# AIR-DISCOVER/Omni-PQ

Measured on AMD Instinct MI355X. Metric: scenes/sec fwd+bwd, 40k-pt ScanNet clouds, batch 8/GPU, higher is better.
Workload: dtype bf16; 1 GPU; BASELINE configs[1]: PQ_Transformer fwd+bwd, 40000-pt synthetic room scenes, batch 8/GPU, 3 input channels; global_batch=8, points=40000, parallelism=dp1, loss=sum of output means (SURVEY 8d)

## Files before the change

### include/omnipq_sa.h

```cpp
#ifndef OMNIPQ_SA_H
#define OMNIPQ_SA_H
#ifdef __cplusplus
extern "C" {

typedef struct omnipq_row_plan {
  const int *rows_dev;
  const void *row_w;
  const int *goff;
  long long rows;
  int gs;
  const float *pool_gamma;
} omnipq_row_plan;

#endif

int omnipq_sa_gather(int b, int n, int m, int s, int cin, int kpad, float inv_radius, const float *xyz,
                     const float *new_xyz, const int *idx, const void *feat_pm, void *X, const omnipq_row_plan *plan, void *stream);

int omnipq_sa_scatter(int b, int n, int m, int s, int cin, int kpad, float inv_radius, const int *idx,
                      const void *dX, float *dfeat_pm, float *dxyz, float *dnew_xyz, void *stream);

int omnipq_sa_build_csr(int b, int n, int m, int s, const int *idx, int *offsets, int *order, int *scratch,
                        const omnipq_row_plan *plan, void *stream);
int omnipq_sa_scatter_csr(int b, int n, int m, int s, int cin, int kpad, float inv_radius, const int *offsets,
// ... 59 lines not shown
                                      float *running_mean, float *running_var, const float *conv_bias, float *a_out,
                                      float *b_out, float *mean_out, float *invstd_out, const void *B, int ldb, void *C,
                                      int ldc, const float *bias, double *sums, float *workspace, int s, void *ymax,
                                      void *ymin, unsigned char *amax, unsigned char *amin, const omnipq_row_plan *plan, void *stream);
int omnipq_sa_pool_select(long long BM, int C, const void *ymax, const void *ymin, const unsigned char *amax,
                          const unsigned char *amin, const float *a, const float *bshift, float *out_f32, void *out_pm,
                          unsigned char *arg, void *ysel, void *stream);
int omnipq_sa_pool_select_finalize(long long BM, int C, const void *ymax, const void *ymin, const unsigned char *amax,
                                   const unsigned char *amin, const double *sums, double count, const float *gamma,
                                   const float *beta, float eps, float momentum, float *running_mean, float *running_var,
                                   float *a_out, float *b_out, float *mean_out, float *invstd_out, float *out_f32,
                                   void *out_pm, unsigned char *arg, void *ysel, const omnipq_row_plan *plan, void *stream);

int omnipq_sa_pool_bwd_stats_sel(long long BM, int C, const void *ysel, const float *mean, const float *invstd,
                                 const float *g_out, const void *out_pm, double *sums, int zeroed, void *stream);
int omnipq_sa_pool_bwd_stats_sel_hot(long long BM, int C, const void *ysel, const float *mean, const float *invstd,
                                     const float *g_out, const void *out_pm, double *sums, int zeroed, const float *a,
                                     const unsigned char *arg, unsigned *hot, void *stream);
int omnipq_gemm_tn_e16_affine(int M, int N, int P, const void *A, int lda, const void *B, int ldb, const float *ba,
                               const float *bb, float *C, float *workspace, float *colsum, const omnipq_row_plan *plan, void *stream);
int omnipq_gemm_tn_grouped(int nprob, const void *probs, float *workspace, void *stream);
int omnipq_gemm_nt_e16_f32(int M, int N, int K, const void *A, int lda, const void *B, int ldb, float *C, int ldc,
                            void *stream);
long long omnipq_sa_l1_rows_workspace_bytes(int b, int m, int s, int C);
int omnipq_sa_l1_rows(int b, int n, int m, int s, int C, float inv_radius, const float *xyz, const float *new_xyz,
                      const int *idx, const float *Z, const void *W1x, int ldw, const int *rows_dev, const int *unit_src,
                      const unsigned char *row_w, void *Y, void *Xrel, double *sums, void *workspace, void *tickets,
                      void *stream);
int omnipq_sa_scatter_rows_csr(int b, int n, int m, int s, int C, float inv_radius, const int *offsets, const int *order,
                               const void *dY, const void *dXr, const int *goff, int gs, float *dfeat32, void *dfeat16,
                               float *dxyz, float *dnew_xyz, void *stream);
void omnipq_tn_debug(int flags);
void omnipq_gemm_nt_small_tile_limit(int tiles);
int omnipq_tn_occupancy(int which);

int omnipq_sa_ball_plan(long long balls, int nsample, int gs, const int *idx, int *goff, int *rows_dev, void *row_w,
                        int *scratch, void *stream);
int omnipq_sa_ball_plan_src(long long balls, int nsample, int gs, const int *idx, int *goff, int *rows_dev, void *row_w,
                            int *unit_src, int *scratch, void *stream);

long long omnipq_gemm_nt_stats_workspace_floats(int M, int N);
int omnipq_gemm_nt_e16_stats(int M, int N, int K, const void *A, int lda, const void *B, int ldb, void *C,
                              int ldc, const float *bias, double *sums, float *workspace, const omnipq_row_plan *plan, void *stream);

int omnipq_gemm_nt_e16_bnbwd(int M, int N, int K, const void *A, int lda, const void *B, int ldb, void *C,
                              int ldc, const void *Y, const float *a, const float *b, const float *mean,
                              const float *invstd, double *sums, float *workspace, const omnipq_row_plan *plan, void *stream);

int omnipq_sa_xyz_moments(long long P, const void *X0, int ldx, double *mom, const omnipq_row_plan *plan, void *stream);
int omnipq_sa_xyz_stats(int C, const void *W0, int ldw0, const double *mom, double *sums, void *stream);
int omnipq_gemm_nt_e16_xyz_bnaffine(int M, int N, int K, const void *X0, int ldx, const void *W0, int ldw0,
                                     const double *fin_sums, double count, const float *gamma, const float *beta,
                                     float eps, float momentum, float *running_mean, float *running_var, float *a_out,
                                     float *b_out, float *mean_out, float *invstd_out, const void *B, int ldb, void *C,
                                     int ldc, double *sums, float *workspace, const omnipq_row_plan *plan, void *stream);
long long omnipq_gemm_nt_xyz_workspace_floats(int M, int N);
int omnipq_gemm_nt_e16_xyz_bnbwd(int M, int N, int K, const void *A, int lda, const void *B, int ldb, const void *X0,
                                  int ldx, const void *W0, int ldw0, const float *a, const float *b, const float *mean,
                                  const float *invstd, double *sums5, float *workspace, const omnipq_row_plan *plan, void *stream);
int omnipq_gemm_tn_e16_xyz_affine(int M, int N, int P, const void *A, int lda, const void *X0, int ldx, const void *W0,
                                   int ldw0, const float *ba, const float *bb, float *C, float *workspace, const omnipq_row_plan *plan, void *stream);
int omnipq_sa_xyz_bwd(int C, const void *W0, int ldw0, const double *mom, const double *sums5, const float *a,
                      const float *mean, const float *invstd, double inv_count, float *dW, void *stream);

int omnipq_colstats(long long P, int C, const void *Y, double *sums, void *stream);
int omnipq_colstats_z(long long P, int C, const void *Y, double *sums, void *stream);
// ... 105 lines not shown
```

### omni-pq_amd/csrc/gemm_bf16.hip

```cpp
#include <atomic>
#include <type_traits>

#include "common.h"

namespace omnipq {

typedef float f32x16 __attribute__((ext_vector_type(16)));
typedef float f32x4 __attribute__((ext_vector_type(4)));

constexpr int GBM = 128, GBN = 128, GBK = 32;
constexpr int GPITCH = 40;

struct GemmArgs {
  int M, N, K;
  int lda, ldb, ldc;
  int k_chunk;
  int m_tiles, n_tiles;
  int relu = 0;
  unsigned drop_thresh = 0, drop_salt = 0;
  float drop_keep_inv = 1.f;
  const unsigned long long *drop_seed = nullptr;
  const int *rows_dev = nullptr;
  const unsigned char *row_w = nullptr;
  int no_store = 0;
};
#ifndef OMNIPQ_DZ_WGS
#define OMNIPQ_DZ_WGS 3
#endif

__device__ __forceinline__ uint4 ldg16(const e16_t *p) { return *reinterpret_cast<const uint4 *>(p); }

#ifdef OMNIPQ_NT_TRACE
__device__ long long g_nt_trace[4096 * 8];
__device__ long long g_nt_real[4096 * 2];
__device__ __forceinline__ long long nt_now() {
  long long t;
  asm volatile("s_waitcnt vmcnt(0) lgkmcnt(0)\n\ts_memtime %0\n\ts_waitcnt lgkmcnt(0)" : "=s"(t) : : "memory");
  return t;
}
#define NT_STAMP(slot)                                                                    \
  {                                                                                       \
    const long long now_ = nt_now();                                                      \
    if (threadIdx.x == 0 && blockIdx.x < 4096) g_nt_trace[blockIdx.x * 8 + (slot)] = now_; \
    if ((slot) == 0 || (slot) == 7) {                                                     \
      const long long real_ = (long long)__builtin_amdgcn_s_memrealtime();                \
      if (threadIdx.x == 0 && blockIdx.x < 4096) g_nt_real[blockIdx.x * 2 + ((slot) == 7)] = real_; \
    }                                                                                     \
  }
#else
#define NT_STAMP(slot)
#endif

struct BnBwdEpilogue {
  const e16_t *Y;
  const float *a, *b, *mean, *invstd;
};

// ... 132 lines not shown
      dzw[i] = (float)g.row_w[ar];
      dzpf[i] = dz.unit_src[ar >> 3] * 8 + (ar & 7);
    }
  }

  f32x16 acc[NI][NI];
#pragma unroll
  for (int i = 0; i < NI; ++i)
#pragma unroll
    for (int j = 0; j < NI; ++j)
#pragma unroll
      for (int r = 0; r < 16; ++r) acc[i][j][r] = 0.f;

  float x0r[NI][3];
  if (XG == 2) {
    for (int c = tid; c < g.N; c += 256) {
      const uint2 w = *reinterpret_cast<const uint2 *>(xg.W0 + (size_t)c * xg.ldw);
      *w0_at(c) = f32x4{e16_lo(w.x), e16_hi(w.x),
                      e16_lo(w.y), 0.f};
    }
    __syncthreads();
  }
  if (XG == 1) {
#pragma unroll
    for (int i = 0; i < NI; ++i) {
      int ar = m0 + srow[i];
      ar = ar < Meff ? ar : Meff - 1;
      const uint2 v = *reinterpret_cast<const uint2 *>(xg.X0 + (size_t)ar * xg.ldx);
      x0r[i][0] = e16_lo(v.x);
      x0r[i][1] = e16_hi(v.x);
      x0r[i][2] = e16_lo(v.y);
    }
  }
  if (AFF) {
    const bool first = bid == 0 && blockIdx.z == 0;
    const int kaff = DZ ? g.K - GBK : g.K;
    for (int c = tid; c < kaff; c += 256) {
      float av, bv;
      if (aff.sums) {
        const double mu = aff.sums[c] / aff.count;
        double var = aff.sums[g.K + c] / aff.count - mu * mu;
        if (var < 0) var = 0;
        const float is = (float)(1.0 / sqrt(var + (double)aff.eps));
        av = aff.gamma[c] * is;
        bv = aff.beta[c] - (float)mu * av;
        if (first) {
          aff.a_out[c] = av;
          aff.b_out[c] = bv;
          aff.mean_out[c] = (float)mu;
          aff.invstd_out[c] = is;
          if (aff.running_mean) {
            const double unbiased = aff.count > 1 ? var * aff.count / (aff.count - 1) : var;
            const float shift = aff.conv_bias ? aff.conv_bias[c] : 0.f;
            aff.running_mean[c] = (1.f - aff.momentum) * aff.running_mean[c] + aff.momentum * ((float)mu + shift);
            aff.running_var[c] = (1.f - aff.momentum) * aff.running_var[c] + aff.momentum * (float)unbiased;
          }
        }
      } else {
        av = aff.a[c];
        bv = aff.b[c];
      }
      if (!PADW0) {
        *aff_at(0, c) = av;
        *aff_at(1, c) = bv;
      }
      if (XG == 1) {
        const uint2 w = *reinterpret_cast<const uint2 *>(xg.W0 + (size_t)c * xg.ldw);
// ... 66 lines not shown
        RA[i_].w = affine_relu_pair(RA[i_].w, fa4_[1][2], fb4_[1][2], fa4_[1][3], fb4_[1][3]);          \
      }                                                                                                 \
      }                                                                                                 \
    }                                                                                                   \
    _Pragma("unroll") for (int i_ = 0; i_ < NI; ++i_) {                                                 \
      *reinterpret_cast<uint4 *>(sa_ + srow[i_] * GPITCH + skc[i_] * 8) = RA[i_];                       \
      *reinterpret_cast<uint4 *>(sb_ + srow[i_] * GPITCH + skc[i_] * 8) = RB[i_];                       \
    }                                                                                                   \
  }

  const int frow = lane & 31, fk = (lane >> 5) * 8;
  auto mma_step = [&](int buf) {
    const e16_t *sa = stage + buf * (2 * T * GPITCH);
    const e16_t *sb = sa + T * GPITCH;
#pragma unroll
    for (int kk = 0; kk < 2; ++kk) {
      e16x8 fa[NI], fb[NI];
#pragma unroll
      for (int i = 0; i < NI; ++i) {
        fa[i] = *reinterpret_cast<const e16x8 *>(sa + (wm * (T / 2) + i * 32 + frow) * GPITCH + kk * 16 + fk);
        fb[i] = *reinterpret_cast<const e16x8 *>(sb + (wn * (T / 2) + i * 32 + frow) * GPITCH + kk * 16 + fk);
      }
#pragma unroll
      for (int i = 0; i < NI; ++i)
#pragma unroll
        for (int j = 0; j < NI; ++j)
          acc[i][j] = mfma_e16_32x32x16(fa[i], fb[j], acc[i][j]);
    }
  };

  if (KRES) {
    const int KP = nk * GBK + 8;
    e16_t *sa = stage, *sb = stage + T * KP;
    uint4 qa[kResMaxSteps], qb[kResMaxSteps];
#pragma unroll
    for (int kt = 0; kt < kResMaxSteps; ++kt)
      if (kt < nk) {
        qa[kt] = ldg16(ga[0] + kt * GBK);
        qb[kt] = ldg16(gb[0] + kt * GBK);
      }
#pragma unroll
    for (int kt = 0; kt < kResMaxSteps; ++kt)
      if (kt < nk) {
        if (AFF) {
          const int k0 = kbeg + kt * GBK + skc[0] * 8;
          const f32x4 fa0 = *reinterpret_cast<const f32x4 *>(aff_at(0, k0)), fa1 = *reinterpret_cast<const f32x4 *>(aff_at(0, k0 + 4));
          const f32x4 fb0 = *reinterpret_cast<const f32x4 *>(aff_at(1, k0));
          const f32x4 fb1 = *reinterpret_cast<const f32x4 *>(aff_at(1, k0 + 4));
          qa[kt].x = affine_relu_pair(qa[kt].x, fa0[0], fb0[0], fa0[1], fb0[1]);
          qa[kt].y = affine_relu_pair(qa[kt].y, fa0[2], fb0[2], fa0[3], fb0[3]);
          qa[kt].z = affine_relu_pair(qa[kt].z, fa1[0], fb1[0], fa1[1], fb1[1]);
          qa[kt].w = affine_relu_pair(qa[kt].w, fa1[2], fb1[2], fa1[3], fb1[3]);
        }
        *reinterpret_cast<uint4 *>(sa + srow[0] * KP + kt * GBK + skc[0] * 8) = qa[kt];
        *reinterpret_cast<uint4 *>(sb + srow[0] * KP + kt * GBK + skc[0] * 8) = qb[kt];
      }
    __syncthreads();
    const e16_t *pa = sa + (wm * (T / 2) + frow) * KP + fk;
    const e16_t *pb = sb + (wn * (T / 2) + frow) * KP + fk;
    for (int kt = 0; kt < nk; ++kt) {
#pragma unroll
      for (int kk = 0; kk < 2; ++kk) {
        const e16x8 fa = *reinterpret_cast<const e16x8 *>(pa + kt * GBK + kk * 16);
        const e16x8 fb = *reinterpret_cast<const e16x8 *>(pb + kt * GBK + kk * 16);
        acc[0][0] = mfma_e16_32x32x16(fa, fb, acc[0][0]);
      }
    }
    __syncthreads();
  } else {
  if (nk > 0) {
    OMNIPQ_LOAD_TILES(ra, rb, 0)
    OMNIPQ_STORE_TILES(ra, rb, 0, 0)
  }
  __syncthreads();
  NT_STAMP(2);

  for (int kt = 0; kt < nk; ++kt) {
    const int buf = kt & 1;
    if (kt + 1 < nk) OMNIPQ_LOAD_TILES(ra, rb, kt + 1)
    mma_step(buf);
    if (kt + 1 < nk) OMNIPQ_STORE_TILES(ra, rb, buf ^ 1, kt + 1)
    __syncthreads();
  }
  if (DZ) {
    const int nk2 = dz.C3 / GBK;
    unsigned dzt[NI];
    const unsigned *dzh[NI];
    const e16_t *gb2[NI];
#pragma unroll
// ... 91 lines not shown
#pragma unroll
          for (int r = 0; r < 16; r += 2) {
            float mine0 = HAS_BIAS ? acc[i][j][r] + bcol[j] : acc[i][j][r];
            float mine1 = HAS_BIAS ? acc[i][j][r + 1] + bcol[j] : acc[i][j][r + 1];
            if (STATS == 0 && g.relu) {
              mine0 = __builtin_fmaxf(mine0, 0.f);
              mine1 = __builtin_fmaxf(mine1, 0.f);
              if (g.drop_thresh) {
                const unsigned e0 = (unsigned)(m0 + wm * (T / 2) + i * 32 + (r & 3) + 8 * (r >> 2) + crow0) * (unsigned)g.ldc +
                                    (unsigned)(n0 + wn * (T / 2) + j * 32 + ccol);
                mine0 = dec_hash(e0, rd_seed) >= g.drop_thresh ? mine0 * g.drop_keep_inv : 0.f;
                mine1 = dec_hash(e0 + (unsigned)g.ldc, rd_seed) >= g.drop_thresh ? mine1 * g.drop_keep_inv : 0.f;
              }
            }
            const unsigned mine = pack_e16x2(mine0, mine1);
            const unsigned other = (unsigned)__builtin_amdgcn_mov_dpp((int)mine, 0xB1, 0xF, 0xF, true);
            cbase[(i * 32 + (r & 3) + 8 * (r >> 2)) * (CP / 2) + j * 16] = __builtin_amdgcn_perm(other, mine, pair_sel);
          }
    };
    if (bias)
      pack_tile(std::true_type{});
    else
      pack_tile(std::false_type{});
    const e16_t *ct = reinterpret_cast<const e16_t *>(smem);
    __syncthreads();
    NT_STAMP(4);
    e16_t *C = reinterpret_cast<e16_t *>(Cout);
    float cs[8], cs2[8];
#pragma unroll
    for (int e = 0; e < 8; ++e) cs[e] = cs2[e] = 0.f;
    float av[8], bv[8], mu[8], is[8];
    float cx[XG == 2 ? 3 : 1][8];
    f32x4 wcol[XG == 2 ? 8 : 1];
    if (STATS == 3 || STATS == 4) {
      int c0 = n0 + (tid % PIECES) * 8;
      c0 = c0 < g.N ? c0 : 0;
#pragma unroll
      for (int e = 0; e < 8; ++e) {
        av[e] = bn.a[c0 + e];
        bv[e] = bn.b[c0 + e];
        mu[e] = bn.mean[c0 + e];
        is[e] = bn.invstd[c0 + e];
        if (XG == 2) {
          wcol[e] = *w0_at(c0 + e);
          cx[0][e] = cx[1][e] = cx[2][e] = 0.f;
        }
      }
    }
    constexpr int ITERS = T * PIECES / 256;
    uint4 ypre[(STATS >= 3 && XG != 2) ? ITERS : 1];
    if (STATS >= 3 && XG != 2) {
#pragma unroll
      for (int it = 0; it < ITERS; ++it) {
        const int q = tid + it * 256;
        const int row = q / PIECES, piece = q % PIECES;
        int gr = m0 + row, gc = n0 + piece * 8;
        gr = gr < Meff ? gr : Meff - 1;
        gc = gc < g.N ? gc : 0;
        ypre[it] = *reinterpret_cast<const uint4 *>(bn.Y + (size_t)gr * g.ldc + gc);
      }
    }
#pragma unroll
    for (int it = 0; it < ITERS; ++it) {
      const int q = tid + it * 256;
      const int row = q / PIECES, piece = q % PIECES;
      const int gr = m0 + row, gc = n0 + piece * 8;
      if (gr < Meff && gc < g.N) {
        const uint4 v = *reinterpret_cast<const uint4 *>(ct + row * CP + piece * 8);
        if (STATS == 5) {
          const uint4 hv = ypre[it];
          const unsigned w[4] = {v.x, v.y, v.z, v.w}, hw[4] = {hv.x, hv.y, hv.z, hv.w};
          unsigned o[4];
#pragma unroll
          for (int e = 0; e < 4; ++e) {
            const float d0 = e16_lo(w[e]), d1 = e16_hi(w[e]);
            const float h0 = e16_lo(hw[e]), h1 = e16_hi(hw[e]);
            o[e] = pack_e16x2(h0 > 0.f ? d0 * g.drop_keep_inv : 0.f, h1 > 0.f ? d1 * g.drop_keep_inv : 0.f);
          }
          *reinterpret_cast<uint4 *>(C + (size_t)gr * g.ldc + gc) = make_uint4(o[0], o[1], o[2], o[3]);
          continue;
        }
        if (XG != 2 && !((STATS == 1 || STATS == 2) && g.no_store))
          *reinterpret_cast<uint4 *>(C + (size_t)gr * g.ldc + gc) = v;
        if (XG == 2) {
// ... 423 lines not shown
  OMNIPQ_LAUNCH_CHECK();
  const long long n4 = (long long)M * N / 4;
  splitk_reduce_bf16_kernel<<<(unsigned)((n4 + 255) / 256), 256, 0, (hipStream_t)stream>>>(
      n4, N, used, reinterpret_cast<const f32x4 *>(workspace), bias, (e16_t *)C);
  OMNIPQ_LAUNCH_CHECK();
  return OMNIPQ_OK;
}

static int g_small_tile_limit = 256;
extern "C" void omnipq_gemm_nt_small_tile_limit(int tiles) { g_small_tile_limit = tiles; }
static bool gemm_nt_small_tiles(int M, int N) {
  return (long long)((M + 127) / 128) * ((N + 127) / 128) <= g_small_tile_limit;
}

static void plan_rows(omnipq::GemmArgs &g) {
  const omnipq::RowPlan &rp = omnipq::row_plan();
  if (rp.rows_dev && rp.rows == g.M && g.m_tiles > kStatsDirectTiles) {
    g.rows_dev = rp.rows_dev;
    g.row_w = rp.row_w;
  }
}

static int stats_reduce(const omnipq::GemmArgs &g, int ns, float *workspace, double *sums, void *stream) {
  int slabs = g.m_tiles / 64;
  if (slabs > 128) slabs = 128;
  if (slabs < 1) slabs = 1;
  omnipq::partial_reduce_kernel<<<dim3((ns * g.N + 255) / 256, slabs), 256, 0, (hipStream_t)stream>>>(
      g.m_tiles, ns * g.N, workspace, sums, g.rows_dev);
  OMNIPQ_LAUNCH_CHECK();
  return OMNIPQ_OK;
}

static bool gemm_nt_kres(int K) { return K <= omnipq::kResMaxSteps * omnipq::GBK; }

static thread_local omnipq::HeldLaunch t_held;
static std::atomic<long long> t_pairs_launched{0};
namespace omnipq {
HeldLaunch &held_launch() { return t_held; }
void count_pair_launch() { ++t_pairs_launched; }
}
struct HeldSmallBlob {
  omnipq::SmallProblem p;
  int lds;
};

static void flush_held() {
  if (t_held.held) omnipq::release_held(t_held);
}

template <int STATS, bool AFF>
static void launch_small_single(const omnipq::SmallProblem &p, int lds, hipStream_t stream) {
  using namespace omnipq;
  auto kern = gemm_nt_kernel<false, STATS, AFF, 64, 0, true>;
  static const hipError_t prepared = hipFuncSetAttribute(reinterpret_cast<const void *>(kern),
                                                         hipFuncAttributeMaxDynamicSharedMemorySize, 96 * 1024);
  (void)prepared;
  kern<<<gemm_nt_grid(p.g), 256, lds, stream>>>(p.g, p.A, p.B, p.C, p.bias, p.stats, p.bn, p.aff, PoolOut(), XyzGen(), DzGen());
}

template <int STATS, bool AFF>
static void held_single(const void *blob, hipStream_t stream) {
  HeldSmallBlob q;
  __builtin_memcpy(&q, blob, sizeof(q));
  launch_small_single<STATS, AFF>(q.p, q.lds, stream);
}

// ... 2 lines not shown
  using namespace omnipq;
  if (n == 2) {
    auto kern = gemm_nt_pair_kernel<STATS, AFF>;
    static const hipError_t prepared = hipFuncSetAttribute(reinterpret_cast<const void *>(kern),
                                                           hipFuncAttributeMaxDynamicSharedMemorySize, 96 * 1024);
    (void)prepared;
    const int n0 = (int)gemm_nt_grid(q[0].p.g).x, n1 = (int)gemm_nt_grid(q[1].p.g).x;
    kern<<<dim3(n0 + n1), 256, q[0].lds > q[1].lds ? q[0].lds : q[1].lds, stream>>>(q[0].p, q[1].p, n0);
    return 1;
  }
  if constexpr (!AFF && (STATS == 0 || STATS == 3)) {
    auto kern = gemm_nt_group_kernel<STATS, AFF>;
    static const hipError_t prepared = hipFuncSetAttribute(reinterpret_cast<const void *>(kern),
                                                           hipFuncAttributeMaxDynamicSharedMemorySize, 96 * 1024);
    (void)prepared;
    NtGroupArgs a;
    a.n = n;
    int wgs = 0, lds = 0;
    for (int i = 0; i < n; ++i) {
      const SmallProblem &p = q[i].p;
      a.item[i] = NtGroupItem{p.g, p.A, p.B, p.C, p.bias, p.stats, p.bn, wgs};
      wgs += (int)gemm_nt_grid(p.g).x;
      lds = q[i].lds > lds ? q[i].lds : lds;
    }
    kern<<<dim3(wgs), 256, lds, stream>>>(a);
    return 1;
  } else {
    for (int i = 0; i < n; ++i) launch_small_single<STATS, AFF>(q[i].p, q[i].lds, stream);
    return 0;
  }
}

template <int STATS, bool AFF>
static void launch_small(const omnipq::GemmArgs &g, const void *A, const void *B, void *C, const float *bias, void *stats,
                         const omnipq::BnBwdEpilogue &bn, const omnipq::AffineIn &aff, void *stream) {
  using namespace omnipq;
  if (gemm_nt_kres(g.K)) {
    int lds = 2 * 64 * (g.K + 8) * 2;
    if (lds < 20480) lds = 20480;
    const HeldSmallBlob q{SmallProblem{g, (const e16_t *)A, (const e16_t *)B, C, bias, stats, bn, aff}, lds};
    const bool consumed = hold_or_pair(
        q, STATS * 2 + (AFF ? 1 : 0), (hipStream_t)stream, &held_single<STATS, AFF>,
        [&](const HeldSmallBlob *recs, int n) { return launch_small_group<STATS, AFF>(recs, n, (hipStream_t)stream); });
    if (!consumed) launch_small_single<STATS, AFF>(q.p, lds, (hipStream_t)stream);
  } else {
    flush_held();
    gemm_nt_kernel<false, STATS, AFF, 64><<<gemm_nt_grid(g), 256, 0, (hipStream_t)stream>>>(
        g, (const e16_t *)A, (const e16_t *)B, C, bias, stats, bn, aff, PoolOut(), XyzGen());
  }
}

extern "C" void omnipq_pair_hold(void) {
  if (!t_held.held || t_held.group) t_held.armed = true;
}

extern "C" int omnipq_pair_group(int n) {
  flush_held();
  t_held.armed = false;
  t_held.group = 0;
  if (n < 1 || n > omnipq::kHeldMax) return OMNIPQ_EINVAL;
  t_held.group = n;
  return OMNIPQ_OK;
}

extern "C" int omnipq_pair_held(void) { return t_held.held; }

extern "C" long long omnipq_pair_flush(void) {
  flush_held();
  t_held.armed = false;
  t_held.group = 0;
// ... 399 lines not shown
```

### omni-pq_amd/pointnet2/rows_mlp.py

```python
import collections
import ctypes
import functools
import os
import typing

import torch

import dropout_state
import sa_fused
from sa_fused import E16, _call, _gemm_nt_bnbwd, _gemm_nt_stats, _gemm_tn, _lib, _p, _round_up, _world, prep_weight, unprep_wgrad, zeros_f32

_FUSE_ACT = True


class Layer:

    def __init__(self, weight, bias=None, bn=None, relu_dropout=None):
        self.weight, self.bias, self.bn, self.relu_dropout = weight, bias, bn, relu_dropout


def enabled():
    return os.environ.get("OMNIPQ_ROWS", "rows") != "torch"


# ... 67 lines not shown
def stack_route(training, N, cin, layers, no_grad=False):
    if no_grad and not training and EVAL_CHAIN and len(layers) >= 2 and \
            all(cout % 32 == 0 for cout, kind in layers if kind == "bn") and \
            eval_chain_ok(cin, tuple(_round_up(cout, 32) for cout, _ in layers)):
        return StackRoute(False, tuple(LayerRoute(kind, "lds" if l else "input", "chain", "folded" if kind == "bn" else "",
                                                  "epilogue" if kind == "act" else "", "", "", "")
                                       for l, (_, kind) in enumerate(layers)))
    L, K, out = len(layers), _round_up(cin, 32), []
    for l, (cout, kind) in enumerate(layers):
        Cp = _round_up(cout, 32)
        feed = "input" if l == 0 else "yab" if out[-1].finalize == "consumer" else "stored"
        if kind == "bn" and training:
            gemm = "stats"
        elif kind == "act" and feed != "yab" and _FUSE_ACT and K < 1024 and N * Cp < (1 << 32):
            gemm = "relu_dropout"
        else:
            gemm = "plain"
        finalize = ""
        if kind == "bn":
            finalize = "running" if not training else \
                "consumer" if (l < L - 1 and sa_fused.affine_pays(N, layers[l + 1][0])) else "launch"
        below = layers[l - 1][1] if l else None
        dgrad = "input" if l == 0 else "bnbwd" if below == "bn" else \
            "mask" if (below == "act" and _FUSE_ACT and Cp < 1024) else "plain"
        out.append(LayerRoute(kind, feed, gemm, finalize, "" if kind != "act" else "epilogue" if gemm == "relu_dropout" else "pass",
                              dgrad, "" if kind != "bn" else "above" if l < L - 1 else "own", ""))
        K = Cp
    for l, r in enumerate(out):
        if r.kind == "act":
            out[l] = r._replace(bwd_act="above" if (l < L - 1 and out[l + 1].dgrad == "mask") else "pass")
    return StackRoute(bool(training), tuple(out))


class _L:
    __slots__ = ("act", "K", "C", "Cp", "Wp", "Wt", "wk", "a", "b", "mean", "invstd", "Y", "X", "has_bias", "fin")


def _hold(lead):
    if lead:
        _lib.omnipq_pair_hold()


def _drain(gen):
    assert not _lib.omnipq_pair_held(), "rows_mlp: a held pair launch leaked into a lone stack"
    try:
        while True:
            next(gen)
    except StopIteration as done:
        return done.value


def _lockstep(*gens):
    n = len(gens)
    out = [None] * n
    alive = [True] * n
    assert not _lib.omnipq_pair_held(), "rows_mlp: a pair launch was still held when a lockstep run started"
    outer, sa_fused.PairStats.active = sa_fused.PairStats.active, sa_fused.PairStats() if n == 2 else None
    try:
        while any(alive):
            if n > 2:
                _lib.omnipq_pair_group(sum(alive))
            for i in range(n):
                if not alive[i]:
                    continue
                held = _lib.omnipq_pair_held()
                try:
                    next(gens[i])
                except StopIteration as done:
                    out[i], alive[i] = done.value, False
                if i < n - 1 and _lib.omnipq_pair_held() != held + 1:
                    _lib.omnipq_pair_flush()
            _lib.omnipq_pair_flush()
    finally:
        sa_fused.PairStats.active = outer
        _lib.omnipq_pair_flush()
    assert not _lib.omnipq_pair_held()
    return out


class _Ctx:
    __slots__ = ("route", "layers", "X0", "geom", "wshapes", "nbias", "targets", "in_dtype", "padded")



def _input_rows(x, N, cin, K):
    cached = getattr(x, "omnipq_rows_in", None)
    if cached is not None and cached[0] == x._version and cached[1].shape == (N, K):
        return cached[1]
    if K == cin:
        X = x.detach().to(E16.dtype).contiguous()
    elif x.dtype in (torch.float32, E16.dtype) and x.stride(1) == 1:
        X = torch.empty((N, K), device=x.device, dtype=E16.dtype)
        _call(_lib.omnipq_pad_rows_e16, x, N, cin, K, x.stride(0), _p(x), int(x.dtype == torch.float32), _p(X))
    else:
        X = torch.nn.functional.pad(x.detach().to(E16.dtype), (0, K - cin))
    if X.data_ptr() != x.data_ptr() and not x.requires_grad:
        try:
            x.omnipq_rows_in = (x._version, X)
        except Exception:
            pass
    return X


def _new_layer(W, bias, K, act, training):
    lay = _L()
    W2 = W.detach().reshape(W.shape[0], -1)
    lay.C, lay.wk = W2.shape
    lay.K, lay.Cp = K, _round_up(lay.C, 32)
    lay.has_bias, lay.act, lay.fin = bias is not None, act, None
    lay.Wp, lay.Wt = prep_weight(W2, lay.Cp, K, transpose=training, persistent=sa_fused.is_persistent(W))
    return lay


def _padded_bias(bias, Cp):
# ... 68 lines not shown
    world = _world() if (training and spec.sync) else 1
    route = stack_route(training, N, cin, tuple((params[4 * l].shape[0], _kind(spec.layers[l])) for l in range(L)))
    X0 = X = _input_rows(x, N, cin, _round_up(cin, 32))
    K = X.shape[1]
    layers = []
    for l, r in enumerate(route.layers):
        W, bias, gamma, beta = params[4 * l:4 * l + 4]
        lay = _new_layer(W, bias, K, spec.layers[l] if r.kind == "act" else None, training)
        if r.kind == "bn" and lay.Cp != lay.C:
            raise RuntimeError("RowsMLP: BatchNorm widths must be multiples of 32")
        sums, slot = sa_fused.pair_sums(lead, 2, lay.C, dev, world) if r.gemm == "stats" else (None, None)
        bp = _padded_bias(bias, lay.Cp) if (lay.has_bias and r.kind != "bn") else None
        _hold(lead)
        lay.Y = _GEMM[r.gemm](lay, X, layers[-1] if r.feed == "yab" else None, N, bp, sums)
        yield
        if r.kind == "bn":
            if training:
                sa_fused.pair_allreduce(sums, slot, lead, world)
            X = _FINALIZE[r.finalize](lay, N, float(N) * world, sums, spec.layers[l], bias, gamma, beta)
            if training:
                sa_fused.bump(spec.layers[l].num_batches_tracked)
        else:
            if r.act == "pass":
                _call(_lib.omnipq_relu_dropout, lay.Y, N * lay.Cp, _p(lay.Y), lay.act.p, _p(lay.act.seed), lay.act.salt)
            X = lay.X = lay.Y
        K = lay.Cp
        layers.append(lay)
    ctx.route, ctx.layers, ctx.X0, ctx.geom = route, layers, X0, (N, cin, world)
    ctx.wshapes = [tuple(params[4 * l].shape) for l in range(L)]
    ctx.nbias = [0 if params[4 * l + 1] is None else params[4 * l + 1].shape[0] for l in range(L)]
    ctx.targets = [(sa_fused.grad_target(params[4 * l]),
                    None if params[4 * l + 1] is None else sa_fused.grad_target(params[4 * l + 1]))
                   for l in range(L)] if training else None
    ctx.in_dtype, ctx.padded = x.dtype, spec.padded
    last = layers[-1]
    return X if (spec.padded or last.Cp == last.C) else X[:, :last.C]



def _layer_kind(lay):
    return "bn" if lay.bn is not None else "act" if lay.relu_dropout is not None else "plain"


def _chain_route(x, layers, training):
    if training or torch.is_grad_enabled() or x.dim() != 2:
        return None
    route = stack_route(False, x.shape[0], x.shape[1], tuple((lay.weight.shape[0], _layer_kind(lay)) for lay in layers), no_grad=True)
    return route if route.layers[0].gemm == "chain" else None


def _infer(x, layers, route, padded):
    global eval_chain_uses
    N, cin = x.shape
    x = x.detach()
    if x.dtype not in (torch.float32, E16.dtype) or x.stride(1) != 1:
        x = x.to(E16.dtype).contiguous()
    L = len(layers)
    recs = (_InferLayer * L)()
    keep = []
    K = _round_up(cin, 32)
    for lay, r, rec in zip(layers, route.layers, recs):
        nl = _new_layer(lay.weight, lay.bias, K, None, False)
        if r.kind == "bn":
            bn = lay.bn
            vecs = [v.detach().float().contiguous() for v in (bn.weight, bn.bias, bn.running_mean, bn.running_var)]
            rec.gamma, rec.beta, rec.running_mean, rec.running_var = (v.data_ptr() for v in vecs)
# ... 40 lines not shown
    wt, bt = ctx.targets[l] if (dfr is not None and ctx.targets is not None) else (None, None)
    if wt is not None and needs_input_grad[3 + 4 * l] and (
            not want_bias or (sa_fused.bias_target_ok(bt, lay.C, lay.Cp) and needs_input_grad[4 + 4 * l])):
        dfr.add(dcur, Xin, lay.Cp, lay.K, N, wt, sa_fused.Crop(lay.C, lay.wk), bt if want_bias else None, below)
        return
    bsum = None
    if want_bias:
        bsum = zeros_f32(lay.Cp, dcur.device)
        grads[4 * l + 1] = bsum[:ctx.nbias[l]]
    dWp = _gemm_tn(dcur, Xin, lay.Cp, lay.K, N, colsum=bsum, below=below)
    grads[4 * l] = unprep_wgrad(dWp, lay.C, lay.wk, 0, ctx.wshapes[l])


def _dgrad_bnbwd(lay, under, dcur, N, sums):
    return _gemm_nt_bnbwd(dcur, lay.Wt, N, lay.K, lay.Cp, under, sums)


def _dgrad_mask(lay, under, dcur, N, sums):
    dprev = torch.empty((N, lay.K), device=dcur.device, dtype=E16.dtype)
    _call(_lib.omnipq_gemm_nt_e16_mask, dcur, N, lay.K, lay.Cp, _p(dcur), lay.Cp, _p(lay.Wt), lay.Cp, _p(dprev), lay.K,
          _p(under.Y), under.act.p)
    return dprev


def _dgrad_plain(lay, under, dcur, N, sums):
    dprev = torch.empty((N, lay.K), device=dcur.device, dtype=E16.dtype)
    sa_fused.gemm_nt_into(dcur, lay.Wt, dprev, N, lay.K, lay.Cp)
    return dprev


_DGRAD = {"bnbwd": _dgrad_bnbwd, "mask": _dgrad_mask, "plain": _dgrad_plain, "input": _dgrad_plain}


def _backward_program(ctx, lead, g, needs_input_grad):
    route, layers = ctx.route, ctx.layers
    if not route.training and any(r.kind == "bn" for r in route.layers):
        raise RuntimeError("RowsMLP: backward through eval-mode BatchNorm is not supported")
    N, cin, world = ctx.geom
    L = len(layers)
    dev = g.device
    grads = [None] * (4 * L)
    dcur, owned = _output_grad(g, layers[-1], N, ctx.padded)
    dx = None
    sums = slot = None
    dfr = sa_fused.deferred_wgrads.active
    for l in range(L - 1, -1, -1):
        lay, r = layers[l], route.layers[l]
        below = layers[l - 1] if r.feed == "yab" else None
        Xin = ctx.X0 if r.feed == "input" else layers[l - 1].Y if r.feed == "yab" else layers[l - 1].X
        if r.kind == "bn":
            if r.bwd_stats == "own":
                sums, slot = sa_fused.pair_sums(lead, 3, lay.C, dev, world)
                _bn_bwd_stats(lay, dcur, N, sums)
                if sa_fused.PairStats.active is not None and (world > 1 or sa_fused._FORCE_COLLECTIVES):
                    yield
            assert sums is not None
            dst = dcur if owned else torch.empty_like(dcur)
            _hold(lead)
            grads[4 * l + 2], grads[4 * l + 3] = sa_fused.bn_backward_apply(dcur, lay, N, lay.C, float(N) * world, sums, world,
                                                                            out=dst, pair=(slot, lead))
            yield
            dcur, owned = dst, True
            if lay.has_bias:
                grads[4 * l + 1] = zeros_f32(lay.C, dev)
        elif r.bwd_act == "pass":
            dst = dcur if owned else torch.empty_like(dcur)
            _act_bwd(lay, dcur, dst, N)
            dcur, owned = dst, True
        _weight_grad(ctx, l, dcur, Xin, below, dfr, needs_input_grad, grads)
        sums = slot = None
        if r.dgrad == "input" and not needs_input_grad[0]:
            break
        if r.dgrad == "bnbwd":
            sums, slot = sa_fused.pair_sums(lead, 3, lay.K, dev, world)
        _hold(lead)
        dprev = _DGRAD[r.dgrad](lay, layers[l - 1] if l else None, dcur, N, sums)
        yield
        if l > 0:
            dcur, owned = dprev, True
        else:
            dx = dprev[:, :cin].to(ctx.in_dtype)
    ctx.layers = None
    return (dx, None, None, *grads)


class RowsMLP(torch.autograd.Function):
    @staticmethod
    def forward(ctx, x, spec, training, *params):
        ctx.e16 = E16.dtype
        return _drain(_forward_program(ctx, False, x, spec, training, params))

    @staticmethod
    def backward(ctx, g):
        E16.select(ctx.e16)
        return _drain(_backward_program(ctx, False, g, ctx.needs_input_grad))


class RowsMLPPair(torch.autograd.Function):

    @staticmethod
    def forward(ctx, xa, spec_a, xb, spec_b, training, n_a, *params):
        ctx.e16 = E16.dtype
        ctx.a, ctx.b, ctx.n_a = _Ctx(), _Ctx(), n_a
        ctx.set_materialize_grads(False)
        ya, yb = _lockstep(_forward_program(ctx.a, True, xa, spec_a, training, params[:n_a]),
                           _forward_program(ctx.b, False, xb, spec_b, training, params[n_a:]))
        return ya, yb

    @staticmethod
    def backward(ctx, ga, gb):
        E16.select(ctx.e16)
        nig, n_a = ctx.needs_input_grad, ctx.n_a
        nig_a = (nig[0], False, False) + tuple(nig[6:6 + n_a])
        nig_b = (nig[2], False, False) + tuple(nig[6 + n_a:])
        if ga is None and gb is None:
            return (None,) * len(nig)
        if ga is None or gb is None:
            outs = []
            for c, g, n in ((ctx.a, ga, nig_a), (ctx.b, gb, nig_b)):
                outs.append(_drain(_backward_program(c, False, g, n)) if g is not None else (None,) * len(n))
            oa, ob = outs
        else:
            oa, ob = _lockstep(*tape_programs(ctx, ga, gb, nig_a, nig_b))
        return (oa[0], None, ob[0], None, None, None) + tuple(oa[3:]) + tuple(ob[3:])


def _spec_of(x_rows, layers, training, padded):
    spec, params = [], []
    for lay in layers:
        bn = lay.bn
        if bn is None and lay.relu_dropout is not None:
            p = float(lay.relu_dropout) if training else 0.0
            spec.append(ActSpec(p, dropout_state.seed(x_rows.device) if p > 0 else None, dropout_state.next_salt() if p > 0 else 0))
        else:
            spec.append(None if bn is None else
                        BnSpec(bn.running_mean, bn.running_var, bn.num_batches_tracked, float(bn.momentum), float(bn.eps)))
        params += [lay.weight, lay.bias, None if bn is None else bn.weight, None if bn is None else bn.bias]
    bns = [lay.bn for lay in layers if lay.bn is not None]
    sync = bool(bns) and all(bool(sa_fused.bn_syncs(bn)) for bn in bns)
    return StackSpec(tuple(spec), bool(padded), sync), params


def run_pair(xa, layers_a, xb, layers_b, training, padded=False, eval_chain=False):
    if eval_chain:
        ra, rb = _chain_route(xa, layers_a, training), _chain_route(xb, layers_b, training)
        if ra is not None and rb is not None:
            return _infer(xa, layers_a, ra, padded), _infer(xb, layers_b, rb, padded)
    spec_a, params_a = _spec_of(xa, layers_a, training, padded)
    spec_b, params_b = _spec_of(xb, layers_b, training, padded)
    return RowsMLPPair.apply(xa, spec_a, xb, spec_b, bool(training), len(params_a), *params_a, *params_b)


class _Taped:
    saved_tensors = ()

# ... 23 lines not shown
```

### omni-pq_amd/pointnet2/sa_fused.py

```python
import collections
import ctypes
import functools
import os
import threading
import typing
import weakref

import torch
import torch.distributed as dist

import pointnet2_utils
import wgrads
from wgrads import Crop, bias_target_ok, cat_params, grad_target, joint_params

_ext = pointnet2_utils._load_ext()
_lib = _ext._lib
E16 = _ext.E16
if os.environ.get("OMNIPQ_TN_DEBUG"):
    _lib.omnipq_tn_debug(int(os.environ["OMNIPQ_TN_DEBUG"]))


def _p(t):
    return ctypes.c_void_p(t.data_ptr() if t is not None else 0)

# ... 422 lines not shown
        _call(_lib.omnipq_gemm_tn_e16_colsum, A, M, N, P, _p(A), M, _p(B), N, _p(C), _p(ws), _p(colsum))
    return C


_TnProblem = _ext.struct("omnipq_tn_problem")


def empty_f32(shape, device):
    return torch.empty(shape, device=device, dtype=torch.float32)


def _plan_buffer(b, dev):
    shape, device = ((b.numel,), dev) if b.param is None else (b.param.shape, b.param.device)
    if b.kind == "empty":
        return empty_f32(shape, device)
    if b.kind == "pooled":
        return zeros_f32(b.numel, device).view(shape)
    return torch.zeros(shape, device=device, dtype=torch.float32)


class deferred_wgrads:
    active = None

    def __init__(self, on_early_flush=None):
        self.on_early_flush = on_early_flush

    def __enter__(self):
        if deferred_wgrads.active is not None:
            raise RuntimeError("deferred_wgrads blocks do not nest")
        self.items = []
        self.sa_items = []
        self.ln_items = []
        self.dz_items = []
        self.producers = set()
        self._inflight = []
        self._assign = []
        self._side_streams = []
        deferred_wgrads.active = self
        return self

    def _note_producer(self, t):
        if t.is_cuda:
            self.producers.add(torch.cuda.current_stream(t.device))

    def add_layernorm(self, part, blocks, C, gamma, beta):
        self._note_producer(part)
        self.ln_items.append((part, blocks, C, gamma, beta))

    def add(self, dY, X, M, N, P, wt, crop, bt, below=None):
        wgrads._refuse_ddp(wt)
        self._note_producer(dY)
        self.items.append(wgrads.Item(dY, X, M, N, P, wt, crop, bt, None if below is None else (below.a, below.b)))

    def add_sa(self, dY, X, M, N, P, wt, crop, below=None, blk=None):
        wgrads._refuse_ddp(wt)
        self._note_producer(dY)
        self.sa_items.append(wgrads.Item(dY, X, M, N, P, wt, crop, None, None if below is None else (below.a, below.b), blk))

    def add_dz(self, args, wt, stage):
        wgrads._refuse_ddp(wt)
        self._note_producer(args[0])
        self.dz_items.append((args, wt, stage))

    def __exit__(self, et, ev, tb):
        deferred_wgrads.active = None
        global COLLECTIVES_LAST_STEP, _COLLECTIVES_MARK
        COLLECTIVES_LAST_STEP, _COLLECTIVES_MARK = COLLECTIVES - _COLLECTIVES_MARK, COLLECTIVES
        if et is None:
            self._wait_producers(None)
            self.flush()
        for st in self._side_streams:
            torch.cuda.current_stream(st.device).wait_stream(st)
        if et is None:
            for param, g in self._assign:
                self._accumulate(param, g)
        self.items = None
        self.sa_items = None
        self.dz_items = None
        self.ln_items = None
        self._inflight = None
        self._assign = None
        self._side_streams = None
        return False

    def _wait_producers(self, stream):
        for ps in self.producers:
            st = stream if stream is not None else torch.cuda.current_stream(ps.device)
            if ps != st:
                st.wait_stream(ps)

    def flush_on(self, stream):
        if not self.items and not self.ln_items:
            return
        cur = torch.cuda.current_stream(stream.device)
        stream.wait_stream(cur)
        self._wait_producers(stream)
        self._inflight.extend(self.items)
        self._inflight.extend(self.ln_items)
        if stream not in self._side_streams:
            self._side_streams.append(stream)
        with torch.cuda.stream(stream):
            self.flush()
            self.items = []
            self.ln_items = []
            if self.on_early_flush is not None:
                self.on_early_flush(self)

    def _flush_layernorms(self):
        todo, self.ln_items = self.ln_items, []
        for i0 in range(0, len(todo), 32):
            chunk = todo[i0:i0 + 32]
            n = len(chunk)
            dev = chunk[0][0].device
            flat = zeros_f32(sum(2 * it[2] for it in chunk), dev)
            parts = (ctypes.c_void_p * n)(*[it[0].data_ptr() for it in chunk])
            blocks = (ctypes.c_int * n)(*[it[1] for it in chunk])
            chans = (ctypes.c_int * n)(*[it[2] for it in chunk])
            outs, off = (ctypes.c_void_p * n)(), 0
            for i, (_, _, C, gamma, beta) in enumerate(chunk):
                outs[i] = flat.data_ptr() + 4 * off
                self._assign.append((gamma, flat[off:off + C].view(gamma.shape)))
                self._assign.append((beta, flat[off + C:off + 2 * C].view(beta.shape)))
                off += 2 * C
            _call(_lib.omnipq_layernorm_param_reduce, flat, n, parts, blocks, chans, outs)
            self._inflight.extend(chunk)

    def flush(self):
        if self.ln_items:
            self._flush_layernorms()
        if self.items:
            self._flush_items(self.items)
        if deferred_wgrads.active is None:
            self._flush_sa()

    def _flush_sa(self):
        if self.sa_items:
            items, self.sa_items = self.sa_items, []
            with _tagged("@sa"):
                self._flush_items(items)
            self._inflight.extend(items)
        if self.dz_items:
            todo, self.dz_items = self.dz_items, []
            for args, wt, stage in todo:
                Y2, below, hot, plan, S, C3, C2, P, alpha, beta, Wp = args
                with _tagged("@sa", stage), _row_plan(plan, P):
                    buf = last_wgrad_dz(Y2, below, hot, plan, S, C3, C2, P, alpha, beta, Wp)
                self._assign.append((wt.param, buf.view(wt.param.shape)))
            self._inflight.extend(todo)

    def _flush_items(self, items):
        dev = items[0].dY.device
        plan = wgrads.place(items)
        bufs = [_plan_buffer(b, dev) for b in plan.buffers]

        def span(s):
            return bufs[s.buf].view(-1)[s.off:s.off + s.n]

        probs = (_TnProblem * len(items))()
        for q, it, pr in zip(probs, items, plan.problems):
            q.rows_dev = 0 if it.blk is None else it.blk.rows_dev.data_ptr()
# ... 868 lines not shown
```

Measured before the change: 1080 scenes/s.

## Defer leaf RowsMLP backwards to end of backward and prefetch K-resident GEMM operands

Two independent changes. In the K-resident small GEMM, operand tiles, BN-affine statistics and epilogue Y/scale values are now loaded into registers before the affine-parameter computation and its barrier, so global-load latency overlaps that setup. In Python, the backward of leaf RowsMLP stacks (no input gradient, single device) is deferred to an autograd end-of-backward callback, and several stacks are run together in lockstep groups so their small launches can be paired. The deferral adds bookkeeping for parameter-gradient assignment and stream producers, and the register prefetch raises register pressure, which may reduce occupancy.

```diff
diff --git a/include/omnipq_sa.h b/include/omnipq_sa.h
--- a/include/omnipq_sa.h
+++ b/include/omnipq_sa.h
@@ -115,6 +115,7 @@
                                float *dxyz, float *dnew_xyz, void *stream);
 void omnipq_tn_debug(int flags);
 void omnipq_gemm_nt_small_tile_limit(int tiles);
+void omnipq_gemm_nt_kres_overlap(int on);
 int omnipq_tn_occupancy(int which);
 
 int omnipq_sa_ball_plan(long long balls, int nsample, int gs, const int *idx, int *goff, int *rows_dev, void *row_w,
diff --git a/omni-pq_amd/csrc/gemm_bf16.hip b/omni-pq_amd/csrc/gemm_bf16.hip
--- a/omni-pq_amd/csrc/gemm_bf16.hip
+++ b/omni-pq_amd/csrc/gemm_bf16.hip
@@ -23,6 +23,7 @@
   const int *rows_dev = nullptr;
   const unsigned char *row_w = nullptr;
   int no_store = 0;
+  int kres_overlap = 0;
 };
 #ifndef OMNIPQ_DZ_WGS
 #define OMNIPQ_DZ_WGS 3
@@ -221,7 +222,102 @@
       x0r[i][2] = e16_lo(v.y);
     }
   }
-  if (AFF) {
+  constexpr int KQ = kResMaxSteps;
+  constexpr bool KEPI = KRES && STATS == 3;
+  const bool kres_early = KRES && g.kres_overlap;
+  uint4 qa[KQ], qb[KQ];
+  float eav[KEPI ? 8 : 1], ebv[KEPI ? 8 : 1], emu[KEPI ? 8 : 1], eis[KEPI ? 8 : 1];
+  uint4 eypre[KEPI ? T * (T / 8) / 256 : 1];
+  constexpr int NC = AFF ? (kResMaxSteps * GBK + 255) / 256 : 1;
+  double ts0[NC], ts1[NC];
+  float tg[NC], tb[NC], trm[NC], trv[NC], tcb[NC];
+  if (AFF && KRES && kres_early) {
+    const bool first = bid == 0 && blockIdx.z == 0;
+#pragma unroll
+    for (int i = 0; i < NC; ++i) {
+      const int c = tid + i * 256;
+      tcb[i] = 0.f;
+      if (c < g.K) {
+        if (aff.sums) {
+          ts0[i] = aff.sums[c];
+          ts1[i] = aff.sums[g.K + c];
+          tg[i] = aff.gamma[c];
+          tb[i] = aff.beta[c];
+          if (first && aff.running_mean) {
+            trm[i] = aff.running_mean[c];
+            trv[i] = aff.running_var[c];
+            if (aff.conv_bias) tcb[i] = aff.conv_bias[c];
+          }
+        } else {
+          tg[i] = aff.a[c];
+          tb[i] = aff.b[c];
+        }
+      }
+    }
+  }
+  if (KRES && kres_early) {
+#pragma unroll
+    for (int kt = 0; kt < KQ; ++kt)
+      if (kt < nk) {
+        qa[kt] = ldg16(ga[0] + kt * GBK);
+        qb[kt] = ldg16(gb[0] + kt * GBK);
+      }
+    if (KEPI) {
+      int c0 = n0 + (tid % PIECES) * 8;
+      c0 = c0 < g.N ? c0 : 0;
+#pragma unroll
+      for (int it = 0; it < T * PIECES / 256; ++it) {
+        const int q = tid + it * 256;
+        int gr = m0 + q / PIECES, gc = n0 + (q % PIECES) * 8;
+        gr = gr < Meff ? gr : Meff - 1;
+        gc = gc < g.N ? gc : 0;
+        eypre[it] = *reinterpret_cast<const uint4 *>(bn.Y + (size_t)gr * g.ldc + gc);
+      }
+#pragma unroll
+      for (int e = 0; e < 8; ++e) {
+        eav[e] = bn.a[c0 + e];
+        ebv[e] = bn.b[c0 + e];
+        emu[e] = bn.mean[c0 + e];
+        eis[e] = bn.invstd[c0 + e];
+      }
+    }
+  }
+  if (AFF && KRES && kres_early) {
+    const bool first = bid == 0 && blockIdx.z == 0;
+#pragma unroll
+    for (int i = 0; i < NC; ++i) {
+      const int c = tid + i * 256;
+      if (c < g.K) {
+        float av, bv;
+        if (aff.sums) {
+          const double mu = ts0[i] / aff.count;
+          double var = ts1[i] / aff.count - mu * mu;
+          if (var < 0) var = 0;
+          const float is = (float)(1.0 / sqrt(var + (double)aff.eps));
+          av = tg[i] * is;
+          bv = tb[i] - (float)mu * av;
+          if (first) {
+            aff.a_out[c] = av;
+            aff.b_out[c] = bv;
+            aff.mean_out[c] = (float)mu;
+            aff.invstd_out[c] = is;
+            if (aff.running_mean) {
+              const double unbiased = aff.count > 1 ? var * aff.count / (aff.count - 1) : var;
+              const float shift = tcb[i];
+              aff.running_mean[c] = (1.f - aff.momentum) * trm[i] + aff.momentum * ((float)mu + shift);
+              aff.running_var[c] = (1.f - aff.momentum) * trv[i] + aff.momentum * (float)unbiased;
+            }
+          }
+        } else {
+          av = tg[i];
+          bv = tb[i];
+        }
+        *aff_at(0, c) = av;
+        *aff_at(1, c) = bv;
+      }
+    }
+    __syncthreads();
+  } else if (AFF) {
     const bool first = bid == 0 && blockIdx.z == 0;
     const int kaff = DZ ? g.K - GBK : g.K;
     for (int c = tid; c < kaff; c += 256) {
@@ -354,29 +450,35 @@
   if (KRES) {
     const int KP = nk * GBK + 8;
     e16_t *sa = stage, *sb = stage + T * KP;
-    uint4 qa[kResMaxSteps], qb[kResMaxSteps];
-#pragma unroll
-    for (int kt = 0; kt < kResMaxSteps; ++kt)
-      if (kt < nk) {
-        qa[kt] = ldg16(ga[0] + kt * GBK);
-        qb[kt] = ldg16(gb[0] + kt * GBK);
-      }
-#pragma unroll
-    for (int kt = 0; kt < kResMaxSteps; ++kt)
-      if (kt < nk) {
-        if (AFF) {
-          const int k0 = kbeg + kt * GBK + skc[0] * 8;
-          const f32x4 fa0 = *reinterpret_cast<const f32x4 *>(aff_at(0, k0)), fa1 = *reinterpret_cast<const f32x4 *>(aff_at(0, k0 + 4));
-          const f32x4 fb0 = *reinterpret_cast<const f32x4 *>(aff_at(1, k0));
-          const f32x4 fb1 = *reinterpret_cast<const f32x4 *>(aff_at(1, k0 + 4));
-          qa[kt].x = affine_relu_pair(qa[kt].x, fa0[0], fb0[0], fa0[1], fb0[1]);
-          qa[kt].y = affine_relu_pair(qa[kt].y, fa0[2], fb0[2], fa0[3], fb0[3]);
-          qa[kt].z = affine_relu_pair(qa[kt].z, fa1[0], fb1[0], fa1[1], fb1[1]);
-          qa[kt].w = affine_relu_pair(qa[kt].w, fa1[2], fb1[2], fa1[3], fb1[3]);
+    auto store_all = [&]() {
+#pragma unroll
+      for (int kt = 0; kt < kResMaxSteps; ++kt)
+        if (kt < nk) {
+          if (AFF) {
+            const int k0 = kbeg + kt * GBK + skc[0] * 8;
+            const f32x4 fa0 = *reinterpret_cast<const f32x4 *>(aff_at(0, k0)), fa1 = *reinterpret_cast<const f32x4 *>(aff_at(0, k0 + 4));
+            const f32x4 fb0 = *reinterpret_cast<const f32x4 *>(aff_at(1, k0));
+            const f32x4 fb1 = *reinterpret_cast<const f32x4 *>(aff_at(1, k0 + 4));
+            qa[kt].x = affine_relu_pair(qa[kt].x, fa0[0], fb0[0], fa0[1], fb0[1]);
+            qa[kt].y = affine_relu_pair(qa[kt].y, fa0[2], fb0[2], fa0[3], fb0[3]);
+            qa[kt].z = affine_relu_pair(qa[kt].z, fa1[0], fb1[0], fa1[1], fb1[1]);
+            qa[kt].w = affine_relu_pair(qa[kt].w, fa1[2], fb1[2], fa1[3], fb1[3]);
+          }
+          *reinterpret_cast<uint4 *>(sa + srow[0] * KP + kt * GBK + skc[0] * 8) = qa[kt];
+          *reinterpret_cast<uint4 *>(sb + srow[0] * KP + kt * GBK + skc[0] * 8) = qb[kt];
         }
-        *reinterpret_cast<uint4 *>(sa + srow[0] * KP + kt * GBK + skc[0] * 8) = qa[kt];
-        *reinterpret_cast<uint4 *>(sb + srow[0] * KP + kt * GBK + skc[0] * 8) = qb[kt];
-      }
+    };
+    if (kres_early) {
+      store_all();
+    } else {
+#pragma unroll
+      for (int kt = 0; kt < kResMaxSteps; ++kt)
+        if (kt < nk) {
+          qa[kt] = ldg16(ga[0] + kt * GBK);
+          qb[kt] = ldg16(gb[0] + kt * GBK);
+        }
+      store_all();
+    }
     __syncthreads();
     const e16_t *pa = sa + (wm * (T / 2) + frow) * KP + fk;
     const e16_t *pb = sb + (wn * (T / 2) + frow) * KP + fk;
@@ -534,7 +636,13 @@
     float av[8], bv[8], mu[8], is[8];
     float cx[XG == 2 ? 3 : 1][8];
     f32x4 wcol[XG == 2 ? 8 : 1];
-    if (STATS == 3 || STATS == 4) {
+    if (KEPI && kres_early) {
+#pragma unroll
+      for (int e = 0; e < 8; ++e) {
+        const int s = KEPI ? e : 0;
+        av[e] = eav[s], bv[e] = ebv[s], mu[e] = emu[s], is[e] = eis[s];
+      }
+    } else if (STATS == 3 || STATS == 4) {
       int c0 = n0 + (tid % PIECES) * 8;
       c0 = c0 < g.N ? c0 : 0;
 #pragma unroll
@@ -551,7 +659,10 @@
     }
     constexpr int ITERS = T * PIECES / 256;
     uint4 ypre[(STATS >= 3 && XG != 2) ? ITERS : 1];
-    if (STATS >= 3 && XG != 2) {
+    if (KEPI && kres_early) {
+#pragma unroll
+      for (int it = 0; it < ITERS; ++it) ypre[KEPI ? it : 0] = eypre[KEPI ? it : 0];
+    } else if (STATS >= 3 && XG != 2) {
 #pragma unroll
       for (int it = 0; it < ITERS; ++it) {
         const int q = tid + it * 256;
@@ -1041,6 +1152,8 @@
 }
 
 static bool gemm_nt_kres(int K) { return K <= omnipq::kResMaxSteps * omnipq::GBK; }
+static int g_kres_overlap = 1;
+extern "C" void omnipq_gemm_nt_kres_overlap(int on) { g_kres_overlap = on != 0; }
 
 static thread_local omnipq::HeldLaunch t_held;
 static std::atomic<long long> t_pairs_launched{0};
@@ -1109,10 +1222,12 @@
 }
 
 template <int STATS, bool AFF>
-static void launch_small(const omnipq::GemmArgs &g, const void *A, const void *B, void *C, const float *bias, void *stats,
+static void launch_small(const omnipq::GemmArgs &g_in, const void *A, const void *B, void *C, const float *bias, void *stats,
                          const omnipq::BnBwdEpilogue &bn, const omnipq::AffineIn &aff, void *stream) {
   using namespace omnipq;
+  GemmArgs g = g_in;
   if (gemm_nt_kres(g.K)) {
+    g.kres_overlap = g_kres_overlap;
     int lds = 2 * 64 * (g.K + 8) * 2;
     if (lds < 20480) lds = 20480;
     const HeldSmallBlob q{SmallProblem{g, (const e16_t *)A, (const e16_t *)B, C, bias, stats, bn, aff}, lds};
diff --git a/omni-pq_amd/pointnet2/rows_mlp.py b/omni-pq_amd/pointnet2/rows_mlp.py
--- a/omni-pq_amd/pointnet2/rows_mlp.py
+++ b/omni-pq_amd/pointnet2/rows_mlp.py
@@ -123,6 +123,18 @@
     return StackRoute(bool(training), tuple(out))
 
 
+DEFER_LEAF_BACKWARD = True
+_LEAF_GROUP_MAX = 14
+
+
+def leaf_backward_route(defer, block, input_grad, targets_ok, ddp_refused, world, force_collectives):
+    if not (defer and block) or input_grad or not targets_ok or ddp_refused:
+        return "now"
+    if world != 1 or force_collectives:
+        return "now"
+    return "deferred"
+
+
 class _L:
     __slots__ = ("act", "K", "C", "Cp", "Wp", "Wt", "wk", "a", "b", "mean", "invstd", "Y", "X", "has_bias", "fin")
 
@@ -170,7 +182,7 @@
 
 
 class _Ctx:
-    __slots__ = ("route", "layers", "X0", "geom", "wshapes", "nbias", "targets", "in_dtype", "padded")
+    __slots__ = ("route", "layers", "X0", "geom", "wshapes", "nbias", "targets", "in_dtype", "padded", "leaf")
 
 
 
@@ -305,6 +317,8 @@
     ctx.targets = [(sa_fused.grad_target(params[4 * l]),
                     None if params[4 * l + 1] is None else sa_fused.grad_target(params[4 * l + 1]))
                    for l in range(L)] if training else None
+    ctx.leaf = [tuple(params[4 * l + 1:4 * l + 4]) if r.kind == "bn" else None for l, r in enumerate(route.layers)] \
+        if training else None
     ctx.in_dtype, ctx.padded = x.dtype, spec.padded
     last = layers[-1]
     return X if (spec.padded or last.Cp == last.C) else X[:, :last.C]
@@ -411,7 +425,7 @@
 _DGRAD = {"bnbwd": _dgrad_bnbwd, "mask": _dgrad_mask, "plain": _dgrad_plain, "input": _dgrad_plain}
 
 
-def _backward_program(ctx, lead, g, needs_input_grad):
+def _backward_program(ctx, lead, g, needs_input_grad, dfr=None):
     route, layers = ctx.route, ctx.layers
     if not route.training and any(r.kind == "bn" for r in route.layers):
         raise RuntimeError("RowsMLP: backward through eval-mode BatchNorm is not supported")
@@ -422,7 +436,7 @@
     dcur, owned = _output_grad(g, layers[-1], N, ctx.padded)
     dx = None
     sums = slot = None
-    dfr = sa_fused.deferred_wgrads.active
+    dfr = dfr if dfr is not None else sa_fused.deferred_wgrads.active
     for l in range(L - 1, -1, -1):
         lay, r = layers[l], route.layers[l]
         below = layers[l - 1] if r.feed == "yab" else None
@@ -463,6 +477,66 @@
     return (dx, None, None, *grads)
 
 
+
+def _leaf_targets_ok(ctx, nig):
+    if ctx.targets is None or ctx.leaf is None:
+        return False
+    for l, (lay, r) in enumerate(zip(ctx.layers, ctx.route.layers)):
+        wt, bt = ctx.targets[l]
+        if wt is None or not nig[3 + 4 * l]:
+            return False
+        if r.kind == "bn":
+            for j, p in enumerate(ctx.leaf[l]):
+                if p is not None and not (isinstance(p, torch.nn.Parameter) and p.requires_grad and nig[4 + 4 * l + j]):
+                    return False
+        elif lay.has_bias and not (sa_fused.bias_target_ok(bt, lay.C, lay.Cp) and nig[4 + 4 * l]):
+            return False
+    return True
+
+
+def _leaf_ddp_refused(ctx):
+    ids = sa_fused.wgrads._DDP_PARAM_IDS
+    if not ids:
+        return False
+    params = [p for wt, bt in ctx.targets for t in (wt, bt) if t is not None for p in t.params]
+    params += [p for leaf in ctx.leaf if leaf is not None for p in leaf if p is not None]
+    return any(id(p) in ids for p in params)
+
+
+def _leaf_deferred(ctxs, nigs):
+    dfr = sa_fused.deferred_wgrads.active
+    for c, nig in zip(ctxs, nigs):
+        block = dfr is not None and c.targets is not None
+        if leaf_backward_route(DEFER_LEAF_BACKWARD, block, nig[0], block and _leaf_targets_ok(c, nig),
+                               block and _leaf_ddp_refused(c), max(c.geom[2], _world()),
+                               sa_fused._FORCE_COLLECTIVES) != "deferred":
+            return None
+    return dfr
+
+
+class LeafBackward(typing.NamedTuple):
+    ctx: object
+    g: torch.Tensor
+    nig: tuple
+    e16: object
+
+
+def run_leaf_backwards(dfr, leaves):
+    before = int(_lib.omnipq_pair_flush())
+    for i0 in range(0, len(leaves), _LEAF_GROUP_MAX):
+        chunk = leaves[i0:i0 + _LEAF_GROUP_MAX]
+        E16.select(chunk[0].e16)
+        progs = [_backward_program(lf.ctx, i + 1 < len(chunk), lf.g, lf.nig, dfr) for i, lf in enumerate(chunk)]
+        outs = _lockstep(*progs) if len(progs) > 1 else [_drain(progs[0])]
+        for lf, out in zip(chunk, outs):
+            for l, leaf in enumerate(lf.ctx.leaf):
+                for j, p in enumerate(leaf or ()):
+                    gp = out[3 + 4 * l + 1 + j]
+                    if p is not None and gp is not None:
+                        dfr.assign(p, gp.view(p.shape))
+    return int(_lib.omnipq_pair_flush()) - before
+
+
 class RowsMLP(torch.autograd.Function):
     @staticmethod
     def forward(ctx, x, spec, training, *params):
@@ -472,7 +546,12 @@
     @staticmethod
     def backward(ctx, g):
         E16.select(ctx.e16)
-        return _drain(_backward_program(ctx, False, g, ctx.needs_input_grad))
+        nig = ctx.needs_input_grad
+        dfr = _leaf_deferred((ctx,), (nig,))
+        if dfr is not None:
+            dfr.add_leaves([LeafBackward(ctx, g, tuple(nig), ctx.e16)])
+            return (None,) * len(nig)
+        return _drain(_backward_program(ctx, False, g, nig))
 
 
 class RowsMLPPair(torch.autograd.Function):
@@ -500,6 +579,10 @@
                 outs.append(_drain(_backward_program(c, False, g, n)) if g is not None else (None,) * len(n))
             oa, ob = outs
         else:
+            dfr = _leaf_deferred((ctx.a, ctx.b), (nig_a, nig_b))
+            if dfr is not None:
+                dfr.add_leaves([LeafBackward(ctx.a, ga, nig_a, ctx.e16), LeafBackward(ctx.b, gb, nig_b, ctx.e16)])
+                return (None,) * len(nig)
             oa, ob = _lockstep(*tape_programs(ctx, ga, gb, nig_a, nig_b))
         return (oa[0], None, ob[0], None, None, None) + tuple(oa[3:]) + tuple(ob[3:])
 
diff --git a/omni-pq_amd/pointnet2/sa_fused.py b/omni-pq_amd/pointnet2/sa_fused.py
--- a/omni-pq_amd/pointnet2/sa_fused.py
+++ b/omni-pq_amd/pointnet2/sa_fused.py
@@ -478,6 +478,10 @@
         self.sa_items = []
         self.ln_items = []
         self.dz_items = []
+        self.leaves = []
+        self.leaf_stacks = 0
+        self.leaf_grids = 0
+        self._leaf_callback = False
         self.producers = set()
         self._inflight = []
         self._assign = []
@@ -492,6 +496,30 @@
     def add_layernorm(self, part, blocks, C, gamma, beta):
         self._note_producer(part)
         self.ln_items.append((part, blocks, C, gamma, beta))
+
+    def add_leaves(self, leaves):
+        for lf in leaves:
+            self._note_producer(lf.g)
+        if not self.leaves and not self._leaf_callback:
+            self._leaf_callback = True
+            torch.autograd.Variable._execution_engine.queue_callback(self._end_of_backward)
+        self.leaves.extend(leaves)
+        self.leaf_stacks += len(leaves)
+
+    def _end_of_backward(self):
+        self._leaf_callback = False
+        if deferred_wgrads.active is self and self.leaves:
+            self._wait_producers(None)
+            self._flush_leaves()
+
+    def assign(self, param, g):
+        self._assign.append((param, g))
+
+    def _flush_leaves(self):
+        import rows_mlp
+        todo, self.leaves = self.leaves, []
+        self._inflight.extend((lf.g, lf.ctx.layers, lf.ctx.X0) for lf in todo)
+        self.leaf_grids += rows_mlp.run_leaf_backwards(self, todo)
 
     def add(self, dY, X, M, N, P, wt, crop, bt, below=None):
         wgrads._refuse_ddp(wt)
@@ -521,6 +549,7 @@
             for param, g in self._assign:
                 self._accumulate(param, g)
         self.items = None
+        self.leaves = None
         self.sa_items = None
         self.dz_items = None
         self.ln_items = None
@@ -536,17 +565,17 @@
                 st.wait_stream(ps)
 
     def flush_on(self, stream):
-        if not self.items and not self.ln_items:
+        if not self.items and not self.ln_items and not self.leaves:
             return
         cur = torch.cuda.current_stream(stream.device)
         stream.wait_stream(cur)
         self._wait_producers(stream)
-        self._inflight.extend(self.items)
         self._inflight.extend(self.ln_items)
         if stream not in self._side_streams:
             self._side_streams.append(stream)
         with torch.cuda.stream(stream):
             self.flush()
+            self._inflight.extend(self.items)
             self.items = []
             self.ln_items = []
             if self.on_early_flush is not None:
@@ -572,6 +601,8 @@
             self._inflight.extend(chunk)
 
     def flush(self):
+        if self.leaves:
+            self._flush_leaves()
         if self.ln_items:
             self._flush_layernorms()
         if self.items:
```

After: 1085 scenes/s, median of 6. Within noise of the previous version (+0.5%).
